# pnlybubbles/LumillyRender

Hardware: NVIDIA B200
Metric: Msamples/s (higher is better)
Workload: dtype f32

## Files before the change

lumillyrender_b200/csrc/api.cpp:

```cpp
#include <cuda_runtime.h>

#include <algorithm>
#include <chrono>
#include <cmath>
#include <cstdio>
#include <cstdlib>
#include <cstring>
#include <memory>
#include <mutex>
#include <string>
#include <system_error>
#include <thread>
#include <vector>

#include "common.h"
#include "kernels.h"

namespace lr {

thread_local std::string g_error;
void set_error(const std::string& s) { g_error = s; }
int fail(int code, const std::string& s) { g_error = s; return code; }

static int g_device = -1;
// ... 20 lines not shown
  return e;
}
static void dev_free(void* p) { if (p) cudaFreeAsync(p, 0); }

struct OnDevice {
  int prev = -1;
  explicit OnDevice(int device) {
    int cur = -1;
    if (cudaGetDevice(&cur) == cudaSuccess && cur != device && cudaSetDevice(device) == cudaSuccess) prev = cur;
  }
  ~OnDevice() { if (prev >= 0) cudaSetDevice(prev); }
  OnDevice(const OnDevice&) = delete;
  OnDevice& operator=(const OnDevice&) = delete;
};

static inline float4 mk4(float x, float y, float z, float w) { float4 r; r.x = x; r.y = y; r.z = z; r.w = w; return r; }
static inline float as_float(int32_t i) { float f; std::memcpy(&f, &i, 4); return f; }

}

using namespace lr;

struct LrScene {
  DevScene dev{};
  std::vector<void*> allocs;
  uint64_t h2d_bytes = 0;
  size_t block_bytes = 0;
  int width = 0, height = 0;
  unsigned long long* d_counters = nullptr;
  mutable float* d_film = nullptr; mutable size_t film_floats = 0;
  mutable float* d_film_sq = nullptr; mutable size_t film_sq_floats = 0;
  mutable float* d_partial = nullptr; mutable size_t partial_floats = 0;
  mutable float* d_partial_sq = nullptr; mutable size_t partial_sq_floats = 0;
  mutable uint64_t acc_samples = 0;
  mutable int acc_launches = 0;
  mutable int last_splits = 1;
  mutable float acc_kernel_ms = 0.0f;
  mutable cudaEvent_t ev0 = nullptr, ev1 = nullptr;
  mutable bool ev_pending = false;
  bool has_ggx = false;
  int device = 0, sm_count = 1;
};

extern "C" {

int lr_abi_version(void) { return LR_ABI_VERSION; }
const char* lr_last_error(void) { return g_error.c_str(); }

static int setup_device(int device, int* sm_count) {
  cudaDeviceProp prop;
  const cudaError_t e = cudaGetDeviceProperties(&prop, device);
  if (e != cudaSuccess) return fail(LR_ERR_NO_DEVICE, std::string("cudaGetDeviceProperties: ") + cudaGetErrorString(e));
  *sm_count = std::max(prop.multiProcessorCount, 1);
  cudaMemPool_t pool;
  if (cudaDeviceGetDefaultMemPool(&pool, device) == cudaSuccess) {
    unsigned long long keep = ~0ull;
    cudaMemPoolSetAttribute(pool, cudaMemPoolAttrReleaseThreshold, &keep);
  }
  return LR_OK;
}

int lr_init(int device) {
  int n = 0;
  cudaError_t e = cudaGetDeviceCount(&n);
  if (e != cudaSuccess || n <= 0)
    return fail(LR_ERR_NO_DEVICE, std::string("no CUDA device available (") + (e != cudaSuccess ? cudaGetErrorString(e) : "count = 0") +
// ... 175 lines not shown
    dv.bvh_hi[k] = d->n_nodes > 0 ? std::fmax(d->nodes[0].f[3 + k], d->nodes[0].f[9 + k]) : 0.0f;
  }
  dv.emission_area = area;
  dv.sky_type = d->sky.type;
  dv.sky_color[0] = d->sky.color[0]; dv.sky_color[1] = d->sky.color[1]; dv.sky_color[2] = d->sky.color[2];
  dv.sky_height = d->sky.height;
  dv.sky_longitude_offset = d->sky.longitude_offset;
  dv.cam = d->camera;
  s->width = d->camera.width; s->height = d->camera.height;
  for (int i = 0; i < d->n_materials; i++) s->has_ggx = s->has_ggx || d->materials[i].type == LR_MAT_GGX;
  guard.s = nullptr;
  *out = s;
  return LR_OK;
}

static int lr_scene_create_body(const LrSceneDesc* d, LrScene** out) {
  if (!d || !out) return fail(LR_ERR_INVALID, "null argument");
  *out = nullptr;
  if (int rc = validate_desc(*d)) return rc;
  if (int rc = ensure_device()) return rc;
  return scene_create(d, g_device, g_sm_count, out);
}
int lr_scene_create(const LrSceneDesc* d, LrScene** out) { LR_GUARDED(lr_scene_create_body(d, out)); }

void lr_scene_destroy(LrScene* s) {
  if (!s) return;
  if (s->ev_pending && s->ev1) cudaEventSynchronize(s->ev1);
  const OnDevice on(s->device);
  for (void* p : s->allocs) dev_free(p);
  dev_free(s->d_film);
  dev_free(s->d_film_sq);
  dev_free(s->d_partial);
  dev_free(s->d_partial_sq);
  if (s->ev0) cudaEventDestroy(s->ev0);
  if (s->ev1) cudaEventDestroy(s->ev1);
  delete s;
}

int lr_scene_bytes(const LrScene* s, uint64_t* h2d_bytes) {
  if (!s || !h2d_bytes) return fail(LR_ERR_INVALID, "null argument");
  *h2d_bytes = s->h2d_bytes;
  return LR_OK;
}

struct FilmShard { int index, count; };

static int resolve_params(const LrScene* s, const LrRenderParams* p, DevParams& dp, const FilmShard* shard = nullptr) {
  if (!s || !p) return fail(LR_ERR_INVALID, "null argument");
  if (p->integrator != LR_INTEGRATOR_PT && p->integrator != LR_INTEGRATOR_PT_DIRECT)
    return fail(LR_ERR_INVALID, "Unknown integrator type");
  if (p->spp_count <= 0 || p->spp_begin < 0) return fail(LR_ERR_INVALID, "spp range must be non-empty and non-negative");
  if (p->depth < 0 || p->depth_limit < 0) return fail(LR_ERR_INVALID, "depth and depth_limit must be >= 0");
  dp.integrator = p->integrator;
  dp.spp_begin = p->spp_begin; dp.spp_count = p->spp_count;
  dp.depth = p->depth; dp.depth_limit = p->depth_limit; dp.no_direct_emitter = p->no_direct_emitter ? 1 : 0;
  dp.seed = p->seed;
  if (p->crop_w > 0) {
    if (p->crop_h <= 0 || p->crop_x < 0 || p->crop_y < 0 || p->crop_x + p->crop_w > s->width || p->crop_y + p->crop_h > s->height)
      return fail(LR_ERR_INVALID, "crop window outside the film");
    dp.crop_x = p->crop_x; dp.crop_y = p->crop_y; dp.crop_w = p->crop_w; dp.crop_h = p->crop_h;
  } else {
    dp.crop_x = 0; dp.crop_y = 0; dp.crop_w = s->width; dp.crop_h = s->height;
  }
  dp.tiles_x = (dp.crop_w + 7) / 8; dp.tiles_y = (dp.crop_h + 3) / 4;
  int splits = shard ? 1 : p->splits;
  if (const char* e_splits = std::getenv("LR_SPLITS"); e_splits && !shard) splits = std::atoi(e_splits);
  if (splits <= 0) {
    const long long px_threads = (long long)dp.tiles_x * dp.tiles_y * 32;
    const long long target = 2LL * s->sm_count * 2048;
    splits = (int)std::min<long long>((target + px_threads - 1) / px_threads, std::max(1, p->spp_count / 4));
  }
  splits = std::max(1, std::min(splits, p->spp_count));
  const size_t px = (size_t)dp.crop_w * dp.crop_h;
  while (splits > 1 && px * 3 * sizeof(float) * splits > (1ull << 30)) splits--;
  dp.splits = splits;
  dp.shard = shard ? shard->index : 0;
  dp.n_shards = shard ? shard->count : 1;
  dp.unit_tiles = shard_tile_count(dp.tiles_x * dp.tiles_y, dp.shard, dp.n_shards);
  const char* e_di = std::getenv("LR_DEFER_ITERS");
  const char* e_dt = std::getenv("LR_DEFER_THRESH");
  dp.defer_iters = e_di ? std::max(1, std::atoi(e_di)) : 3;
  dp.defer_thresh = e_dt ? std::max(1, std::min(32, std::atoi(e_dt))) : 12;
  const char* e_org = std::getenv("LR_ORGANISATION");
  dp.organisation = !e_org ? 0 : (std::strcmp(e_org, "persistent") == 0 ? 1 : (std::strcmp(e_org, "pool") == 0 ? 2 : 0));

  return LR_OK;
}

static int ensure_scratch(float** buf, size_t* have, size_t need) {
  if (*have >= need) return LR_OK;
  dev_free(*buf);
  *buf = nullptr; *have = 0;
  LR_CUDA(dev_alloc((void**)buf, need * sizeof(float)));
  *have = need;
  return LR_OK;
}

static uint64_t shard_pixels(const DevParams& dp) {
  if (dp.n_shards == 1) return (uint64_t)dp.crop_w * dp.crop_h;
  uint64_t n = 0;
  for (int j = 0; j < dp.unit_tiles; j++) {
    const int t = shard_tile(j, dp.shard, dp.n_shards), tx = t % dp.tiles_x, ty = t / dp.tiles_x;
    n += (uint64_t)std::min(8, dp.crop_w - 8 * tx) * (uint64_t)std::min(4, dp.crop_h - 4 * ty);
  }
  return n;
}

static int accumulate(const LrScene* s, const LrRenderParams* p, float* d_sum, float* d_sumsq, void* cuda_stream, const FilmShard* shard) {
  if (!s) return fail(LR_ERR_INVALID, "null argument");
  const OnDevice on(s->device);
  DevParams dp;
  if (int rc = resolve_params(s, p, dp, shard)) return rc;
  if (!d_sum) return fail(LR_ERR_INVALID, "d_sum is null");
  cudaStream_t st = (cudaStream_t)cuda_stream;
  const size_t n = (size_t)dp.crop_w * dp.crop_h * 3;
  float* ksum = d_sum; float* ksq = d_sumsq;
  if (s->ev_pending) {
    float ms = 0.0f;
    if (cudaEventSynchronize(s->ev1) == cudaSuccess && cudaEventElapsedTime(&ms, s->ev0, s->ev1) == cudaSuccess) s->acc_kernel_ms += ms;
    s->ev_pending = false;
  }
  if (dp.unit_tiles == 0) return LR_OK;
  if (dp.splits > 1) {
    if (int rc = ensure_scratch(&s->d_partial, &s->partial_floats, n * dp.splits)) return rc;
    ksum = s->d_partial;
    if (d_sumsq) {
      if (int rc = ensure_scratch(&s->d_partial_sq, &s->partial_sq_floats, n * dp.splits)) return rc;
      ksq = s->d_partial_sq;
    }
  }
  LR_CUDA(cudaEventRecord(s->ev0, st));
  {
    unsigned int* next_unit = reinterpret_cast<unsigned int*>(s->d_counters + C_NEXT_UNIT);
    LR_CUDA(cudaMemsetAsync(next_unit, 0, sizeof(unsigned long long), st));
    LR_CUDA(launch_render_persistent(s->dev, dp, s->has_ggx, p->count_traversal != 0, ksum, d_sumsq ? ksq : nullptr, s->d_counters, next_unit,
                                     std::max(s->sm_count, 1), st));
    s->acc_launches++;
  }
  if (dp.splits > 1) {
    LR_CUDA(launch_reduce_splits(d_sum, s->d_partial, n, dp.splits, st));
    s->acc_launches++;
    if (d_sumsq) { LR_CUDA(launch_reduce_splits(d_sumsq, s->d_partial_sq, n, dp.splits, st)); s->acc_launches++; }
  }
  LR_CUDA(cudaEventRecord(s->ev1, st));
  s->ev_pending = true;
  s->acc_samples += shard_pixels(dp) * (uint64_t)dp.spp_count;
  s->last_splits = dp.splits;
  return LR_OK;
}

int lr_render_accumulate_device(const LrScene* s, const LrRenderParams* p, float* d_sum, float* d_sumsq, void* cuda_stream) {
  return accumulate(s, p, d_sum, d_sumsq, cuda_stream, nullptr);
}

int lr_stats_fetch(const LrScene* s, void* cuda_stream, LrStats* stats) {
  if (!s || !stats) return fail(LR_ERR_INVALID, "null argument");
  const OnDevice on(s->device);
  cudaStream_t st = (cudaStream_t)cuda_stream;
  LR_CUDA(cudaStreamSynchronize(st));
  if (s->ev_pending) {
    float ms = 0.0f;
    LR_CUDA(cudaEventSynchronize(s->ev1));
    LR_CUDA(cudaEventElapsedTime(&ms, s->ev0, s->ev1));
    s->acc_kernel_ms += ms;
    s->ev_pending = false;
  }
  unsigned long long c[C_COUNT];
  LR_CUDA(cudaMemcpy(c, s->d_counters, sizeof(c), cudaMemcpyDeviceToHost));
  LR_CUDA(cudaMemset(s->d_counters, 0, sizeof(c)));
  std::memset(stats, 0, sizeof(*stats));
  stats->rays = c[C_RAYS]; stats->nonfinite_samples = c[C_NONFINITE]; stats->gate_retraces = c[C_RETRACE];
  stats->nodes_visited = c[C_NODES]; stats->tris_tested = c[C_TRIS]; stats->spheres_tested = c[C_SPHERES];
  stats->flat_tris_tested = c[C_FLAT_TRIS]; stats->flat_boxes_tested = c[C_FLAT_BOXES];
  stats->samples = s->acc_samples; stats->kernel_ms = s->acc_kernel_ms; stats->launches = s->acc_launches; stats->splits = s->last_splits;
  s->acc_samples = 0; s->acc_kernel_ms = 0.0f; s->acc_launches = 0;
  return LR_OK;
}

int lr_render(const LrScene* s, const LrRenderParams* p, float* out_rgb, float* out_sumsq, LrStats* stats) {
  if (!s) return fail(LR_ERR_INVALID, "null argument");
  const OnDevice on(s->device);
  DevParams dp;
  if (int rc = resolve_params(s, p, dp)) return rc;
  if (!out_rgb) return fail(LR_ERR_INVALID, "out_rgb is null");
  const size_t n = (size_t)dp.crop_w * dp.crop_h * 3;
  if (int rc = ensure_scratch(&s->d_film, &s->film_floats, n)) return rc;
  if (out_sumsq) if (int rc = ensure_scratch(&s->d_film_sq, &s->film_sq_floats, n)) return rc;
  float *d_sum = s->d_film, *d_sq = out_sumsq ? s->d_film_sq : nullptr;
  int rc = LR_OK;
  do {
    if (cudaMemsetAsync(d_sum, 0, n * sizeof(float), 0) != cudaSuccess) { rc = fail(LR_ERR_CUDA, "cudaMemsetAsync failed"); break; }
    if (out_sumsq && cudaMemsetAsync(d_sq, 0, n * sizeof(float), 0) != cudaSuccess) { rc = fail(LR_ERR_CUDA, "cudaMemsetAsync failed"); break; }
    LrStats dummy;
    if (stats == nullptr) stats = &dummy;
    if ((rc = lr_stats_fetch(s, nullptr, stats)) != LR_OK) break;
    if ((rc = lr_render_accumulate_device(s, p, d_sum, d_sq, nullptr)) != LR_OK) break;
    cudaError_t e = launch_scale(d_sum, n, (float)dp.spp_count, 0);
    if (e != cudaSuccess) { rc = fail(LR_ERR_CUDA, std::string("scale: ") + cudaGetErrorString(e)); break; }
    if ((rc = lr_stats_fetch(s, nullptr, stats)) != LR_OK) break;
    stats->launches += 1;
    e = cudaMemcpy(out_rgb, d_sum, n * sizeof(float), cudaMemcpyDeviceToHost);
    if (e == cudaSuccess && out_sumsq) e = cudaMemcpy(out_sumsq, d_sq, n * sizeof(float), cudaMemcpyDeviceToHost);
// ... 646 lines not shown
```

lumillyrender_b200/csrc/device_scene.h:

```cpp
#pragma once
#include <cuda_runtime.h>
#include <stdint.h>
#include "../../include/lumilly.h"

namespace lr {

constexpr int kStackDepth = 64;
constexpr int kBlockThreads = 128;

struct DevScene {
  const float4* nodes;
  const float4* tris;
  const float4* tri_box;
  const float4* tri_n;
  const float4* spheres;
  const int2* sphere_meta;
  const float4* mats;
  const float* emitter_cdf;
  const float4* emitters;
  const float4* sky_pixels;
  int n_nodes, n_tris, n_spheres, n_emitters;
  int n_bvh_tris;
  float bvh_lo[3], bvh_hi[3];
  float emission_area;
  int sky_type;
  float sky_color[3];
  int sky_height;
  float sky_longitude_offset;
  LrCamera cam;
};

struct DevParams {
  int integrator;
  int spp_begin, spp_count;
  int depth, depth_limit, no_direct_emitter;
  unsigned long long seed;
  int crop_x, crop_y, crop_w, crop_h;
  int splits;
  int tiles_x, tiles_y;
  int shard, n_shards;
  int unit_tiles;
  int defer_iters, defer_thresh;
  int organisation;
};

__host__ __device__ inline int shard_of_tile(int tile, int n_shards) { return tile % n_shards; }
__host__ __device__ inline int shard_tile(int j, int shard, int n_shards) { return j * n_shards + shard; }
__host__ __device__ inline int shard_tile_count(int n_tiles, int shard, int n_shards) {
  return shard < n_tiles ? (n_tiles - shard + n_shards - 1) / n_shards : 0;
}
__host__ __device__ inline int shard_device(int shard, int n_devices) { return shard % n_devices; }
__host__ __device__ inline unsigned int render_units(const DevParams& p) { return (unsigned int)p.unit_tiles * 32u * (unsigned int)p.splits; }

enum CounterSlot { C_RAYS = 0, C_NONFINITE = 1, C_NODES = 2, C_TRIS = 3, C_SPHERES = 4, C_RETRACE = 5, C_FLAT_TRIS = 6, C_NEXT_UNIT = 7, C_FLAT_BOXES = 8, C_COUNT = 9 };

}
```

lumillyrender_b200/csrc/path_vertex.inc:

```
      bool need_new = false;
      bool fetch_unit = false;

      if (ready) {
        if (flags & F_HAS_RAY) {
          int depth = flags & F_DEPTH_MASK;
          bool allow_emission = (flags & F_ALLOW_EMISSION) != 0;
          bool has_shadow_next = false;
          const F3 d = d0;
          if (NR == 2 && (flags & F_HAS_SHADOW)) {
            PV_LOAD_SHADOW();
            if (id1 != -1 && fabsf(t1 - q_dist) <= kEPS) {
              const Surface lf = surface_at(sc, o, d1, t1, id1);
              const float light_cos = dot(-d1, lf.n);
              if (light_cos > 0.0f) {
                const Mat lm = load_mat(sc, lf.mat);
                const float g_term = q_point_cos * light_cos / q_sqr;
                const F3 l_i = lm.emissive ? lm.emission : f3(0.0f, 0.0f, 0.0f);
                const F3 direct = q_brdf * l_i * g_term / q_pdf;
                L = L + q_T * (q_prr != 1.0f ? direct / q_prr : direct);
              }
            }
          }
          bool finish = false;
          if (id0 == -1) {
// ... 55 lines not shown
              float pdf;
              mat_sample(m, wo, sf.n, rng, wi, pdf);
              F3 f_bsdf = f3(0, 0, 0);
#pragma unroll 1
              for (int k = (NR == 2 && has_shadow_next) ? 0 : 1; k < 2; k++) {
                const F3 f = mat_brdf(m, wo, k == 0 ? nee_dir : wi, k == 0 ? pn : sf.n, sf.pos);
                if (k == 0) { q_brdf = f; PV_STORE_QBRDF(); } else f_bsdf = f;
              }
              const F3 coef = mat_coef(m, wo, sf.n, t);
              const float c = dot(wi, sf.n);
              T = T * (f_bsdf * coef * c / pdf);
              if (prr != 1.0f) T = T / prr;
              o = sf.pos;
              d0 = wi;
              if (NR == 2 && has_shadow_next) d1 = nee_dir;
              depth++;
            }
          }
          if (finish) {
            PV_LOAD_FILM();
            const F3 e = (L * cam_g) * cam_w;
            if (!(isfinite(e.x) && isfinite(e.y) && isfinite(e.z))) n_nonfinite++;
            sum = sum + e;
            if (want_sumsq) sumsq = sumsq + e * e;
            un.y += 1;
            need_new = true;
          }
          flags = (flags & ~(F_DEPTH_MASK | F_ALLOW_EMISSION | F_HAS_SHADOW)) | (depth & F_DEPTH_MASK) |
                  (allow_emission ? F_ALLOW_EMISSION : 0) | (has_shadow_next ? F_HAS_SHADOW : 0);
        } else {
          need_new = true;
        }

        if (need_new && (!(flags & F_HAS_UNIT) || un.y >= un.z)) {
          if (flags & F_HAS_UNIT) {
            const size_t pi = (size_t)un.x, n_px = (size_t)p.crop_w * p.crop_h;
            if (p.splits == 1) {
              out_sum[3 * pi + 0] = sum.x; out_sum[3 * pi + 1] = sum.y; out_sum[3 * pi + 2] = sum.z;
              if (want_sumsq) { out_sumsq[3 * pi + 0] = sumsq.x; out_sumsq[3 * pi + 1] = sumsq.y; out_sumsq[3 * pi + 2] = sumsq.z; }
            } else {
              float* ps = out_sum + 3 * (n_px * un.w + pi);
              ps[0] = sum.x; ps[1] = sum.y; ps[2] = sum.z;
              if (want_sumsq) { float* pq = out_sumsq + 3 * (n_px * un.w + pi); pq[0] = sumsq.x; pq[1] = sumsq.y; pq[2] = sumsq.z; }
            }
          }
          fetch_unit = true;
        }
      }

      {
        bool need = fetch_unit;
        while (true) {
          const unsigned m = __ballot_sync(kFull, need);
          if (m == 0u) break;
          const int leader = __ffs(m) - 1;
          unsigned int base = 0;
          if (lane == leader) base = atomicAdd(next_unit, (unsigned int)__popc(m));
          base = __shfl_sync(kFull, base, leader);
          if (need) {
            const unsigned int u = base + (unsigned int)__popc(m & lanemask_lt());
            if (u >= n_units) {
              alive = false;
              need = false;
            } else {
              int lx, ly, split;
              if (decode_unit(p, u, lx, ly, split)) {
                const int per = p.spp_count / p.splits, rem = p.spp_count % p.splits;
                un.x = ly * p.crop_w + lx;
                un.y = p.spp_begin + split * per + min(split, rem);
                un.z = un.y + per + (split < rem ? 1 : 0);
                un.w = split;
                flags |= F_HAS_UNIT;
                sum = f3(0.0f, 0.0f, 0.0f);
                sumsq = f3(0.0f, 0.0f, 0.0f);
                if (p.splits == 1) {
                  const float* ps = out_sum + 3 * (size_t)un.x;
                  sum = f3(ps[0], ps[1], ps[2]);
                  if (want_sumsq) { const float* pq = out_sumsq + 3 * (size_t)un.x; sumsq = f3(pq[0], pq[1], pq[2]); }
                }
                need = false;
              }
            }
          }
        }
      }

      const bool go = ready && alive;
      if (go && need_new) {
        const int lx = un.x % p.crop_w, ly = un.x / p.crop_w;
        const int x = p.crop_x + lx, y = p.crop_y + ly;
        const unsigned int pixel = (unsigned int)(y * sc.cam.width + x);
        rng.seed(p.seed, pixel, (unsigned int)un.y);
        camera_sample_rng(sc.cam, x, y, rng, o, d0, cam_g, cam_w);
        T = f3(1.0f, 1.0f, 1.0f);
        L = f3(0.0f, 0.0f, 0.0f);
        flags = (flags & ~(F_DEPTH_MASK | F_HAS_SHADOW)) | F_ALLOW_EMISSION | F_HAS_RAY;
        PV_STORE_FILM();
      }
#pragma unroll 1
      for (int r = 0; r < NR; r++) {
        const bool on = go && (r == 0 || (flags & F_HAS_SHADOW));
        if (!__any_sync(kFull, on)) continue;
        if (on) {
          const F3 d = r == 0 ? d0 : d1;
          const F3 inv = f3(1.0f / d.x, 1.0f / d.y, 1.0f / d.z);
          float t = 3.0e38f;
          int id = -1;
          flat_hits<COUNT>(sc, flat, o, d, inv, t, id, tc);
          n_rays++;
          const bool pd = TREE && sc.n_nodes > 0 && bvh_bounds_hit(sc, o, inv, t < 3.0e38f ? t * 1.0001f + 1e-4f : 3.0e38f);
          if (r == 0) { t0 = t; id0 = id; pend0 = pd; } else { t1 = t; id1 = id; pend1 = pd; }
        }
      }
```

lumillyrender_b200/csrc/persistent.cuh:

```cuda
#pragma once
#include <algorithm>

#include "device_path.cuh"
#include "kernels.h"

namespace lr {

namespace pk {

constexpr unsigned kFull = 0xffffffffu;
enum { F_DEPTH_MASK = 0xffff, F_ALLOW_EMISSION = 1 << 16, F_HAS_RAY = 1 << 17, F_HAS_SHADOW = 1 << 18, F_HAS_UNIT = 1 << 20 };

LR_DEV unsigned lanemask_lt() { unsigned m; asm("mov.u32 %0, %%lanemask_lt;" : "=r"(m)); return m; }
LR_DEV unsigned int warp_sum_u(unsigned int v) { return __reduce_add_sync(kFull, v); }

LR_DEV bool decode_unit(const DevParams& p, unsigned int u, int& lx, int& ly, int& split) {
  const unsigned int per_split = (unsigned int)p.unit_tiles * 32u;
  split = (int)(u / per_split);
  const unsigned int r = u % per_split;
  const unsigned int tile = (unsigned int)shard_tile((int)(r >> 5), p.shard, p.n_shards), lane = r & 31u;
  lx = (int)(tile % p.tiles_x) * 8 + (int)(lane & 7u);
  ly = (int)(tile / p.tiles_x) * 4 + (int)(lane >> 3);
  return lx < p.crop_w && ly < p.crop_h;
}

template <bool COUNT>
__device__ __noinline__ void trace_strict(const DevScene& sc, F3 o, F3 d, float* t, int* id, TraceCounters* tc) {
  trace<COUNT>(sc, o, d, *t, *id, *tc);
}

}

#ifndef LR_MB_PT_TREE
#define LR_MB_PT_TREE 6
#endif
#ifndef LR_MB_PT_FLAT
#define LR_MB_PT_FLAT 8
#endif
#ifndef LR_MB_PTD_TREE
#define LR_MB_PTD_TREE 16
#endif
#ifndef LR_MB_PTD_FLAT
#define LR_MB_PTD_FLAT 4
#endif
template <int INTEGRATOR, bool TREE>
struct MinBlocks {
  static constexpr int value = INTEGRATOR == LR_INTEGRATOR_PT_DIRECT ? (TREE ? LR_MB_PTD_TREE : LR_MB_PTD_FLAT) : (TREE ? LR_MB_PT_TREE : LR_MB_PT_FLAT);
};

template <int INTEGRATOR, bool TREE, bool COUNT, int BUILD>
__global__ void __launch_bounds__(kBlockThreads, MinBlocks<INTEGRATOR, TREE>::value)
render_persistent_kernel(const __grid_constant__ DevScene sc, const __grid_constant__ DevParams p, float* __restrict__ out_sum,
                         float* __restrict__ out_sumsq, unsigned long long* __restrict__ counters, unsigned int* __restrict__ next_unit) {
  using namespace pk;
  constexpr int NR = INTEGRATOR == LR_INTEGRATOR_PT_DIRECT ? 2 : 1;
  const int lane = (int)(threadIdx.x & 31);
  const unsigned int n_units = render_units(p);
  const bool want_sumsq = out_sumsq != nullptr;
  __shared__ __align__(16) float4 flat_tab[kFlatListFloat4];
  __shared__ __align__(8) unsigned long long flat_bar;
  const FlatList flat = stage_flat_list(sc, flat_tab, &flat_bar);

  F3 o = f3(0, 0, 0), T = f3(1, 1, 1), L = f3(0, 0, 0), sum = f3(0, 0, 0), sumsq = f3(0, 0, 0);
  F3 d0 = f3(0, 0, 1), d1 = f3(0, 0, 1);
  float t0 = 3.0e38f, t1 = 3.0e38f;
  int id0 = -1, id1 = -1;
  bool pend0 = false, pend1 = false;
  float cam_g = 1.0f, cam_w = 1.0f;
  int4 un = make_int4(0, 0, 0, 0);
  Pcg rng;
  rng.state = 0;
  F3 q_T = f3(0, 0, 0), q_brdf = f3(0, 0, 0);
  float q_prr = 1.0f, q_point_cos = 0.0f, q_dist = 0.0f, q_sqr = 1.0f, q_pdf = 1.0f;
  int flags = 0;
  bool alive = true;
  unsigned int n_nonfinite = 0, n_retrace = 0, n_rays = 0;
  TraceCounters tc;
  tc.nodes = tc.tris = tc.spheres = tc.flat_tris = tc.flat_boxes = 0;

  while (true) {
    for (int it = 0; it < p.defer_iters; it++) {
      const bool ready = alive && !(pend0 || pend1);
      if (!__any_sync(kFull, ready)) break;
// ... 22 lines not shown
        int id = r == 0 ? id0 : id1;
        bvh_traverse_unified<COUNT>(sc, o, d, inv, t, id, tc);
        if (id >= 0 && id < sc.n_bvh_tris && !bvh_hit_is_gated(sc, o, inv, id)) {
          trace_strict<COUNT>(sc, o, d, &t, &id, &tc);
          n_retrace++;
        }
        if (r == 0) { t0 = t; id0 = id; pend0 = false; } else { t1 = t; id1 = id; pend1 = false; }
      }
    }
    if (!__any_sync(kFull, alive)) break;
  }

  n_rays = warp_sum_u(n_rays);
  n_nonfinite = warp_sum_u(n_nonfinite);
  n_retrace = warp_sum_u(n_retrace);
  if (COUNT) {
    tc.nodes = warp_sum_u(tc.nodes); tc.tris = warp_sum_u(tc.tris); tc.spheres = warp_sum_u(tc.spheres);
    tc.flat_tris = warp_sum_u(tc.flat_tris); tc.flat_boxes = warp_sum_u(tc.flat_boxes);
  }
  if (lane == 0) {
    if (n_rays) atomicAdd(counters + C_RAYS, (unsigned long long)n_rays);
    if (n_nonfinite) atomicAdd(counters + C_NONFINITE, (unsigned long long)n_nonfinite);
    if (n_retrace) atomicAdd(counters + C_RETRACE, (unsigned long long)n_retrace);
    if (COUNT) {
      atomicAdd(counters + C_NODES, (unsigned long long)tc.nodes);
      atomicAdd(counters + C_TRIS, (unsigned long long)tc.tris);
      atomicAdd(counters + C_SPHERES, (unsigned long long)tc.spheres);
      atomicAdd(counters + C_FLAT_TRIS, (unsigned long long)tc.flat_tris);
      atomicAdd(counters + C_FLAT_BOXES, (unsigned long long)tc.flat_boxes);
    }
  }
}

template <int INTEGRATOR, bool TREE, bool COUNT, int BUILD>
cudaError_t launch_persistent_one(const DevScene& sc, const DevParams& p, float* out_sum, float* out_sumsq,
                                  unsigned long long* counters, unsigned int* next_unit, int sm_count, cudaStream_t stream) {
  int nb = 0;
  if (cudaOccupancyMaxActiveBlocksPerMultiprocessor(&nb, render_persistent_kernel<INTEGRATOR, TREE, COUNT, BUILD>, kBlockThreads, 0) !=
          cudaSuccess || nb <= 0) nb = 4;
  const long long units = render_units(p);
  const long long want = (units + kBlockThreads - 1) / kBlockThreads;
  const unsigned int blocks = (unsigned int)std::max<long long>(1, std::min<long long>(want, (long long)nb * sm_count));
  render_persistent_kernel<INTEGRATOR, TREE, COUNT, BUILD><<<blocks, kBlockThreads, 0, stream>>>(sc, p, out_sum, out_sumsq, counters, next_unit);
  return cudaGetLastError();
}

}
```

lumillyrender_b200/csrc/pool.cuh:

```cuda
#pragma once
#include <algorithm>

#include "device_path.cuh"
#include "kernels.h"
#include "persistent.cuh"

namespace lr {

#ifndef LR_POOL_SLOTS
#define LR_POOL_SLOTS 64
#endif
#ifndef LR_POOL_SLOTS_PTD
#define LR_POOL_SLOTS_PTD 48
#endif
#ifndef LR_POOL_BSTART
#define LR_POOL_BSTART 32
#endif
#ifndef LR_PMB_PT_TREE
#define LR_PMB_PT_TREE 6
#endif
#ifndef LR_PMB_PTD_TREE
#define LR_PMB_PTD_TREE 6
#endif

// ... 21 lines not shown
__host__ __device__ constexpr int warp_words(bool want_sumsq) { return words_per_slot<INTEGRATOR>(want_sumsq) * slots<INTEGRATOR>() + 32; }

template <int N>
LR_DEV int select_take(int* list, int lane, unsigned (&words)[N], int quota, int rot) {
  const unsigned lt = pk::lanemask_lt();
  const unsigned bit = 1u << lane;
  int base = 0;
#pragma unroll
  for (int r = 0; r < N; r++) {
    if (r != rot) continue;
#pragma unroll
    for (int k = 0; k < N; k++) {
      const int i = (k + r) % N;
      const unsigned w = words[i];
      const int rank = base + __popc(w & lt);
      const bool mine = (w & bit) != 0u && rank < quota;
      if (mine) list[rank] = i * 32 + lane;
      words[i] = w & ~__ballot_sync(pk::kFull, mine);
      base += __popc(w);
    }
  }
  __syncwarp();
  return min(base, quota);
}

}

template <int INTEGRATOR, bool TREE>
struct PoolMinBlocks {
  static_assert(TREE, "the pool kernel is built for scenes with a BVH only (persistent_inst.cu)");
  static constexpr int value = INTEGRATOR == LR_INTEGRATOR_PT_DIRECT ? LR_PMB_PTD_TREE : LR_PMB_PT_TREE;
};

template <int INTEGRATOR, bool TREE, bool COUNT, int BUILD>
__global__ void __launch_bounds__(kBlockThreads, PoolMinBlocks<INTEGRATOR, TREE>::value)
render_pool_kernel(const __grid_constant__ DevScene sc, const __grid_constant__ DevParams p, float* __restrict__ out_sum,
                   float* __restrict__ out_sumsq, unsigned long long* __restrict__ counters, unsigned int* __restrict__ next_unit) {
  using namespace pk;
  using namespace pl;
  constexpr int NR = INTEGRATOR == LR_INTEGRATOR_PT_DIRECT ? 2 : 1;
  constexpr int NS = slots<INTEGRATOR>();
  constexpr int kWords = mask_words<INTEGRATOR>();
  __shared__ __align__(16) float4 flat_tab[kFlatListFloat4];
  __shared__ __align__(8) unsigned long long flat_bar;
  const FlatList flat = stage_flat_list(sc, flat_tab, &flat_bar);
  extern __shared__ float pool_smem[];
  const int lane = (int)(threadIdx.x & 31);
  const unsigned int n_units = render_units(p);
  const bool want_sumsq = out_sumsq != nullptr;
  float* const pool = pool_smem + (threadIdx.x >> 5) * warp_words<INTEGRATOR>(want_sumsq);
  int* const list = (int*)(pool + words_per_slot<INTEGRATOR>(want_sumsq) * NS);
  constexpr int W_SQ = NR == 2 ? (int)W_PTD_COUNT : (int)W_PT_COUNT;
#define SLF(w) pool[(w) * NS + s]
#define SLI(w) ((int*)pool)[(w) * NS + s]

  for (int s = lane; s < NS; s += 32) SLI(W_FLAGS) = 0;
  __syncwarp();

  unsigned pend[NR * kWords], dead[kWords];
#pragma unroll
  for (int i = 0; i < NR * kWords; i++) pend[i] = 0u;
#pragma unroll
  for (int i = 0; i < kWords; i++) dead[i] = (i + 1) * 32 <= NS ? 0u : ~0u << (NS - i * 32);
  unsigned int n_nonfinite = 0, n_retrace = 0, n_rays = 0;
  TraceCounters tc;
  tc.nodes = tc.tris = tc.spheres = tc.flat_tris = tc.flat_boxes = 0;
  int rot_a = 0, rot_b = 0;

  while (true) {
    unsigned rdy[kWords];
    int nA = 0, nB = 0;
#pragma unroll
    for (int i = 0; i < kWords; i++) {
      rdy[i] = ~(pend[i] | (NR == 2 ? pend[(NR - 1) * kWords + i] : 0u) | dead[i]);
      nA += __popc(rdy[i]);
    }
#pragma unroll
    for (int i = 0; i < NR * kWords; i++) nB += __popc(pend[i]);
    if (nA + nB == 0) break;

    if (!TREE || !(nB >= LR_POOL_BSTART || nB >= nA)) {
      const int n_sel = select_take<kWords>(list, lane, rdy, 32, rot_a);
      rot_a = rot_a + 1 == kWords ? 0 : rot_a + 1;
      const bool ready = lane < n_sel;
      const int s = ready ? list[lane] : 0;
      __syncwarp();
      bool alive = true;
      bool pend0 = false, pend1 = false;

      F3 o = f3(0, 0, 0), T = f3(1, 1, 1), L = f3(0, 0, 0), sum = f3(0, 0, 0), sumsq = f3(0, 0, 0);
      F3 d0 = f3(0, 0, 1), d1 = f3(0, 0, 1);
      float t0 = 3.0e38f, t1 = 3.0e38f;
      int id0 = -1, id1 = -1;
      float cam_g = 1.0f, cam_w = 1.0f;
      int4 un = make_int4(0, 0, 0, 0);
      Pcg rng;
      rng.state = 0;
      F3 q_T = f3(0, 0, 0), q_brdf = f3(0, 0, 0);
      float q_prr = 1.0f, q_point_cos = 0.0f, q_dist = 0.0f, q_sqr = 1.0f, q_pdf = 1.0f;
      int flags = 0;
      if (ready) {
        o = f3(SLF(W_OX), SLF(W_OY), SLF(W_OZ));
        d0 = f3(SLF(W_DX), SLF(W_DY), SLF(W_DZ));
        t0 = SLF(W_T0); id0 = SLI(W_ID0);
        T = f3(SLF(W_TX), SLF(W_TY), SLF(W_TZ));
        L = f3(SLF(W_LX), SLF(W_LY), SLF(W_LZ));
        rng.state = (unsigned long long)(unsigned int)SLI(W_RNGLO) | ((unsigned long long)(unsigned int)SLI(W_RNGHI) << 32);
        flags = SLI(W_FLAGS);
      }
#define PV_LOAD_SHADOW()                                                                                                  \
  do {                                                                                                                    \
    d1 = f3(SLF(W_D1X), SLF(W_D1Y), SLF(W_D1Z));                                                                          \
    t1 = SLF(W_T1); id1 = SLI(W_ID1);                                                                                     \
    q_T = f3(SLF(W_QTX), SLF(W_QTY), SLF(W_QTZ));                                                                         \
// ... 19 lines not shown
    SLF(W_CAMG) = cam_g; SLF(W_CAMW) = cam_w;                                                                             \
    SLI(W_UNX) = un.x; SLI(W_UNY) = un.y; SLI(W_UNZ) = un.z; SLI(W_UNW) = un.w;                                           \
    if (want_sumsq) { SLF(W_SQ) = sumsq.x; SLF(W_SQ + 1) = sumsq.y; SLF(W_SQ + 2) = sumsq.z; }                            \
  } while (0)

#include "path_vertex.inc"

#undef PV_LOAD_SHADOW
#undef PV_STORE_SHADOW
#undef PV_STORE_QBRDF
#undef PV_LOAD_FILM
#undef PV_STORE_FILM
      if (go) {
        SLF(W_OX) = o.x; SLF(W_OY) = o.y; SLF(W_OZ) = o.z;
        SLF(W_DX) = d0.x; SLF(W_DY) = d0.y; SLF(W_DZ) = d0.z;
        SLF(W_T0) = t0; SLI(W_ID0) = id0;
        SLF(W_TX) = T.x; SLF(W_TY) = T.y; SLF(W_TZ) = T.z;
        SLF(W_LX) = L.x; SLF(W_LY) = L.y; SLF(W_LZ) = L.z;
        SLI(W_RNGLO) = (int)(unsigned int)rng.state; SLI(W_RNGHI) = (int)(unsigned int)(rng.state >> 32);
        SLI(W_FLAGS) = flags;
        if (NR == 2 && (flags & F_HAS_SHADOW)) {
          SLF(W_D1X) = d1.x; SLF(W_D1Y) = d1.y; SLF(W_D1Z) = d1.z;
          SLF(W_T1) = t1; SLI(W_ID1) = id1;
        }
      }
      const unsigned bit = 1u << (s & 31);
      const int w = s >> 5;
#pragma unroll
      for (int i = 0; i < kWords; i++) {
        pend[i] |= __reduce_or_sync(kFull, (go && pend0 && w == i) ? bit : 0u);
        if (NR == 2) pend[(NR - 1) * kWords + i] |= __reduce_or_sync(kFull, (go && pend1 && w == i) ? bit : 0u);
        dead[i] |= __reduce_or_sync(kFull, (ready && !alive && w == i) ? bit : 0u);
      }
    } else {
      const int n_sel = select_take<NR * kWords>(list, lane, pend, 32, rot_b);
      rot_b = rot_b + 1 == NR * kWords ? 0 : rot_b + 1;
      if (lane < n_sel) {
        const int item = list[lane];
        const int s = item % (32 * kWords);
        const bool shadow = NR == 2 && item >= 32 * kWords;
        const F3 o = f3(SLF(W_OX), SLF(W_OY), SLF(W_OZ));
        const F3 d = shadow ? f3(SLF(W_D1X), SLF(W_D1Y), SLF(W_D1Z)) : f3(SLF(W_DX), SLF(W_DY), SLF(W_DZ));
        const F3 inv = f3(1.0f / d.x, 1.0f / d.y, 1.0f / d.z);
        float t = shadow ? SLF(W_T1) : SLF(W_T0);
        int id = shadow ? SLI(W_ID1) : SLI(W_ID0);
        bvh_traverse_unified<COUNT>(sc, o, d, inv, t, id, tc);
        if (id >= 0 && id < sc.n_bvh_tris && !bvh_hit_is_gated(sc, o, inv, id)) {
          trace_strict<COUNT>(sc, o, d, &t, &id, &tc);
          n_retrace++;
        }
        if (shadow) { SLF(W_T1) = t; SLI(W_ID1) = id; } else { SLF(W_T0) = t; SLI(W_ID0) = id; }
      }
    }
    __syncwarp();
  }
#undef SLF
#undef SLI

  n_rays = warp_sum_u(n_rays);
  n_nonfinite = warp_sum_u(n_nonfinite);
  n_retrace = warp_sum_u(n_retrace);
  if (COUNT) {
    tc.nodes = warp_sum_u(tc.nodes); tc.tris = warp_sum_u(tc.tris); tc.spheres = warp_sum_u(tc.spheres);
    tc.flat_tris = warp_sum_u(tc.flat_tris); tc.flat_boxes = warp_sum_u(tc.flat_boxes);
  }
  if (lane == 0) {
    if (n_rays) atomicAdd(counters + C_RAYS, (unsigned long long)n_rays);
    if (n_nonfinite) atomicAdd(counters + C_NONFINITE, (unsigned long long)n_nonfinite);
    if (n_retrace) atomicAdd(counters + C_RETRACE, (unsigned long long)n_retrace);
    if (COUNT) {
      atomicAdd(counters + C_NODES, (unsigned long long)tc.nodes);
      atomicAdd(counters + C_TRIS, (unsigned long long)tc.tris);
      atomicAdd(counters + C_SPHERES, (unsigned long long)tc.spheres);
      atomicAdd(counters + C_FLAT_TRIS, (unsigned long long)tc.flat_tris);
      atomicAdd(counters + C_FLAT_BOXES, (unsigned long long)tc.flat_boxes);
    }
  }
}

template <int INTEGRATOR, bool TREE, bool COUNT, int BUILD>
cudaError_t launch_pool_one(const DevScene& sc, const DevParams& p, float* out_sum, float* out_sumsq, unsigned long long* counters,
                            unsigned int* next_unit, int sm_count, cudaStream_t stream) {
  auto kernel = render_pool_kernel<INTEGRATOR, TREE, COUNT, BUILD>;
  const size_t smem = (size_t)(kBlockThreads / 32) * pl::warp_words<INTEGRATOR>(out_sumsq != nullptr) * sizeof(float);
  cudaError_t e = cudaFuncSetAttribute(kernel, cudaFuncAttributeMaxDynamicSharedMemorySize, (int)smem);
  if (e != cudaSuccess) return e;
  int nb = 0;
  if (cudaOccupancyMaxActiveBlocksPerMultiprocessor(&nb, kernel, kBlockThreads, smem) != cudaSuccess || nb <= 0) nb = 2;
  const long long units = render_units(p);
  const long long per_block = (long long)(kBlockThreads / 32) * pl::slots<INTEGRATOR>();
  const long long want = (units + per_block - 1) / per_block;
  const unsigned int blocks = (unsigned int)std::max<long long>(1, std::min<long long>(want, (long long)nb * sm_count));
  kernel<<<blocks, kBlockThreads, smem, stream>>>(sc, p, out_sum, out_sumsq, counters, next_unit);
  return cudaGetLastError();
}

}
```

Baseline: 1362.

## Chain per-pixel sample chunks with device-side release/acquire instead of split reductions

When only one split is chosen, each pixel's samples are divided into chunks that run as separate work units. Each unit waits on a per-pixel done counter, using acquire and release atomics, before it accumulates into the film. The aim is to expose more parallel units for small images without the partial-buffer reduction pass. The cost is a per-pixel counter memset, spin-waiting lanes, and a timeout path that abandons stalled units.

After: 1428 (median of 6 runs). 4.9% higher.

```diff
diff --git a/lumillyrender_b200/csrc/api.cpp b/lumillyrender_b200/csrc/api.cpp
--- a/lumillyrender_b200/csrc/api.cpp
+++ b/lumillyrender_b200/csrc/api.cpp
@@ -76,6 +76,7 @@
   mutable float* d_film_sq = nullptr; mutable size_t film_sq_floats = 0;
   mutable float* d_partial = nullptr; mutable size_t partial_floats = 0;
   mutable float* d_partial_sq = nullptr; mutable size_t partial_sq_floats = 0;
+  mutable unsigned int* d_done = nullptr; mutable size_t done_words = 0;
   mutable uint64_t acc_samples = 0;
   mutable int acc_launches = 0;
   mutable int last_splits = 1;
@@ -317,6 +318,7 @@
   dev_free(s->d_film_sq);
   dev_free(s->d_partial);
   dev_free(s->d_partial_sq);
+  dev_free(s->d_done);
   if (s->ev0) cudaEventDestroy(s->ev0);
   if (s->ev1) cudaEventDestroy(s->ev1);
   delete s;
@@ -359,6 +361,9 @@
   const size_t px = (size_t)dp.crop_w * dp.crop_h;
   while (splits > 1 && px * 3 * sizeof(float) * splits > (1ull << 30)) splits--;
   dp.splits = splits;
+  const char* e_chunk = std::getenv("LR_CHUNK_SPP");
+  dp.chunk_spp = !e_chunk ? 0 : (std::atoi(e_chunk) > 0 ? std::atoi(e_chunk) : -1);
+  dp.done = nullptr;
   dp.shard = shard ? shard->index : 0;
   dp.n_shards = shard ? shard->count : 1;
   dp.unit_tiles = shard_tile_count(dp.tiles_x * dp.tiles_y, dp.shard, dp.n_shards);
@@ -415,6 +420,13 @@
     }
   }
   LR_CUDA(cudaEventRecord(s->ev0, st));
+  if (dp.splits == 1 && dp.chunk_spp >= 0) {
+    const size_t n_px = (size_t)dp.crop_w * dp.crop_h;
+    static_assert(sizeof(unsigned int) == sizeof(float), "the done counters share the float scratch allocator");
+    if (int rc = ensure_scratch((float**)&s->d_done, &s->done_words, n_px)) return rc;
+    LR_CUDA(cudaMemsetAsync(s->d_done, 0, n_px * sizeof(unsigned int), st));
+    dp.done = s->d_done;
+  }
   {
     unsigned int* next_unit = reinterpret_cast<unsigned int*>(s->d_counters + C_NEXT_UNIT);
     LR_CUDA(cudaMemsetAsync(next_unit, 0, sizeof(unsigned long long), st));
@@ -453,6 +465,9 @@
   unsigned long long c[C_COUNT];
   LR_CUDA(cudaMemcpy(c, s->d_counters, sizeof(c), cudaMemcpyDeviceToHost));
   LR_CUDA(cudaMemset(s->d_counters, 0, sizeof(c)));
+  if (c[C_WAIT_ABANDONED])
+    return fail(LR_ERR_CUDA, std::to_string(c[C_WAIT_ABANDONED]) + " chained render unit(s) waited more than " + std::to_string(kChainWaitMs / 1000) +
+                                 " s for the previous chunk of their pixel and were abandoned: the image is incomplete");
   std::memset(stats, 0, sizeof(*stats));
   stats->rays = c[C_RAYS]; stats->nonfinite_samples = c[C_NONFINITE]; stats->gate_retraces = c[C_RETRACE];
   stats->nodes_visited = c[C_NODES]; stats->tris_tested = c[C_TRIS]; stats->spheres_tested = c[C_SPHERES];
diff --git a/lumillyrender_b200/csrc/device_scene.h b/lumillyrender_b200/csrc/device_scene.h
--- a/lumillyrender_b200/csrc/device_scene.h
+++ b/lumillyrender_b200/csrc/device_scene.h
@@ -42,6 +42,8 @@
   int unit_tiles;
   int defer_iters, defer_thresh;
   int organisation;
+  unsigned int* done;
+  int chunk_spp;
 };
 
 __host__ __device__ inline int shard_of_tile(int tile, int n_shards) { return tile % n_shards; }
@@ -51,7 +53,31 @@
 }
 __host__ __device__ inline int shard_device(int shard, int n_devices) { return shard % n_devices; }
 __host__ __device__ inline unsigned int render_units(const DevParams& p) { return (unsigned int)p.unit_tiles * 32u * (unsigned int)p.splits; }
+__host__ __device__ inline bool decode_unit(const DevParams& p, unsigned int u, int& lx, int& ly, int& split) {
+  const unsigned int per_split = (unsigned int)p.unit_tiles * 32u;
+  split = (int)(u / per_split);
+  const unsigned int r = u % per_split;
+  const unsigned int tile = (unsigned int)shard_tile((int)(r >> 5), p.shard, p.n_shards), lane = r & 31u;
+  lx = (int)(tile % p.tiles_x) * 8 + (int)(lane & 7u);
+  ly = (int)(tile / p.tiles_x) * 4 + (int)(lane >> 3);
+  return lx < p.crop_w && ly < p.crop_h;
+}
+__host__ __device__ inline void split_samples(const DevParams& p, int split, int& begin, int& end) {
+  const int per = p.spp_count / p.splits, rem = p.spp_count % p.splits;
+  begin = p.spp_begin + split * per + (split < rem ? split : rem);
+  end = begin + per + (split < rem ? 1 : 0);
+}
 
-enum CounterSlot { C_RAYS = 0, C_NONFINITE = 1, C_NODES = 2, C_TRIS = 3, C_SPHERES = 4, C_RETRACE = 5, C_FLAT_TRIS = 6, C_NEXT_UNIT = 7, C_FLAT_BOXES = 8, C_COUNT = 9 };
+__host__ __device__ inline int chain_chunks(const DevParams& p, long long slots) {
+  if (p.chunk_spp > 0) return (p.spp_count + p.chunk_spp - 1) / p.chunk_spp;
+  const long long px = (long long)p.unit_tiles * 32;
+  if (px < slots) return 1;
+  const long long want = (64 * slots + px - 1) / px, most = p.spp_count / 64;
+  return (int)(want < most ? want : most > 1 ? most : 1);
+}
+
+enum CounterSlot { C_RAYS = 0, C_NONFINITE = 1, C_NODES = 2, C_TRIS = 3, C_SPHERES = 4, C_RETRACE = 5, C_FLAT_TRIS = 6, C_NEXT_UNIT = 7, C_FLAT_BOXES = 8,
+                   C_WAIT_ABANDONED = 9, C_COUNT = 10 };
+constexpr unsigned int kChainWaitMs = 20000;
 
 }
diff --git a/lumillyrender_b200/csrc/path_vertex.inc b/lumillyrender_b200/csrc/path_vertex.inc
--- a/lumillyrender_b200/csrc/path_vertex.inc
+++ b/lumillyrender_b200/csrc/path_vertex.inc
@@ -111,12 +111,13 @@
           need_new = true;
         }
 
-        if (need_new && (!(flags & F_HAS_UNIT) || un.y >= un.z)) {
+        if (need_new && !(CHAIN && (flags & F_WAIT)) && (!(flags & F_HAS_UNIT) || un.y >= un.z)) {
           if (flags & F_HAS_UNIT) {
             const size_t pi = (size_t)un.x, n_px = (size_t)p.crop_w * p.crop_h;
-            if (p.splits == 1) {
+            if (p.splits == 1 || CHAIN) {
               out_sum[3 * pi + 0] = sum.x; out_sum[3 * pi + 1] = sum.y; out_sum[3 * pi + 2] = sum.z;
               if (want_sumsq) { out_sumsq[3 * pi + 0] = sumsq.x; out_sumsq[3 * pi + 1] = sumsq.y; out_sumsq[3 * pi + 2] = sumsq.z; }
+              if (CHAIN) st_release(p.done + pi, (unsigned int)un.w + 1u);
             } else {
               float* ps = out_sum + 3 * (n_px * un.w + pi);
               ps[0] = sum.x; ps[1] = sum.y; ps[2] = sum.z;
@@ -144,15 +145,16 @@
             } else {
               int lx, ly, split;
               if (decode_unit(p, u, lx, ly, split)) {
-                const int per = p.spp_count / p.splits, rem = p.spp_count % p.splits;
                 un.x = ly * p.crop_w + lx;
-                un.y = p.spp_begin + split * per + min(split, rem);
-                un.z = un.y + per + (split < rem ? 1 : 0);
+                split_samples(p, split, un.y, un.z);
                 un.w = split;
                 flags |= F_HAS_UNIT;
                 sum = f3(0.0f, 0.0f, 0.0f);
                 sumsq = f3(0.0f, 0.0f, 0.0f);
-                if (p.splits == 1) {
+                if (CHAIN) {
+                  flags = (flags & ~(F_HAS_RAY | F_HAS_SHADOW)) | F_WAIT;
+                  sum.x = __uint_as_float(timer_ms());
+                } else if (p.splits == 1) {
                   const float* ps = out_sum + 3 * (size_t)un.x;
                   sum = f3(ps[0], ps[1], ps[2]);
                   if (want_sumsq) { const float* pq = out_sumsq + 3 * (size_t)un.x; sumsq = f3(pq[0], pq[1], pq[2]); }
@@ -164,21 +166,40 @@
         }
       }
 
+      bool waiting = false;
+      if (CHAIN && ready && alive && (flags & F_WAIT)) {
+        if (!fetch_unit) PV_LOAD_FILM();
+        const size_t pi = (size_t)un.x;
+        if (ld_acquire(p.done + pi) == (unsigned int)un.w) {
+          const float* ps = out_sum + 3 * pi;
+          sum = f3(ps[0], ps[1], ps[2]);
+          if (want_sumsq) { const float* pq = out_sumsq + 3 * pi; sumsq = f3(pq[0], pq[1], pq[2]); }
+          flags &= ~F_WAIT;
+        } else if (timer_ms() - __float_as_uint(sum.x) > kChainWaitMs) {
+          atomicAdd(counters + C_WAIT_ABANDONED, 1ull);
+          alive = false;
+        } else {
+          waiting = true;
+        }
+      }
+
       const bool go = ready && alive;
       if (go && need_new) {
-        const int lx = un.x % p.crop_w, ly = un.x / p.crop_w;
-        const int x = p.crop_x + lx, y = p.crop_y + ly;
-        const unsigned int pixel = (unsigned int)(y * sc.cam.width + x);
-        rng.seed(p.seed, pixel, (unsigned int)un.y);
-        camera_sample_rng(sc.cam, x, y, rng, o, d0, cam_g, cam_w);
-        T = f3(1.0f, 1.0f, 1.0f);
-        L = f3(0.0f, 0.0f, 0.0f);
-        flags = (flags & ~(F_DEPTH_MASK | F_HAS_SHADOW)) | F_ALLOW_EMISSION | F_HAS_RAY;
+        if (!waiting) {
+          const int lx = un.x % p.crop_w, ly = un.x / p.crop_w;
+          const int x = p.crop_x + lx, y = p.crop_y + ly;
+          const unsigned int pixel = (unsigned int)(y * sc.cam.width + x);
+          rng.seed(p.seed, pixel, (unsigned int)un.y);
+          camera_sample_rng(sc.cam, x, y, rng, o, d0, cam_g, cam_w);
+          T = f3(1.0f, 1.0f, 1.0f);
+          L = f3(0.0f, 0.0f, 0.0f);
+          flags = (flags & ~(F_DEPTH_MASK | F_HAS_SHADOW)) | F_ALLOW_EMISSION | F_HAS_RAY;
+        }
         PV_STORE_FILM();
       }
 #pragma unroll 1
       for (int r = 0; r < NR; r++) {
-        const bool on = go && (r == 0 || (flags & F_HAS_SHADOW));
+        const bool on = go && !waiting && (r == 0 || (flags & F_HAS_SHADOW));
         if (!__any_sync(kFull, on)) continue;
         if (on) {
           const F3 d = r == 0 ? d0 : d1;
diff --git a/lumillyrender_b200/csrc/persistent.cuh b/lumillyrender_b200/csrc/persistent.cuh
--- a/lumillyrender_b200/csrc/persistent.cuh
+++ b/lumillyrender_b200/csrc/persistent.cuh
@@ -1,5 +1,6 @@
 #pragma once
 #include <algorithm>
+#include <cuda/atomic>
 
 #include "device_path.cuh"
 #include "kernels.h"
@@ -9,19 +10,17 @@
 namespace pk {
 
 constexpr unsigned kFull = 0xffffffffu;
-enum { F_DEPTH_MASK = 0xffff, F_ALLOW_EMISSION = 1 << 16, F_HAS_RAY = 1 << 17, F_HAS_SHADOW = 1 << 18, F_HAS_UNIT = 1 << 20 };
+enum { F_DEPTH_MASK = 0xffff, F_ALLOW_EMISSION = 1 << 16, F_HAS_RAY = 1 << 17, F_HAS_SHADOW = 1 << 18, F_HAS_UNIT = 1 << 20, F_WAIT = 1 << 21 };
 
 LR_DEV unsigned lanemask_lt() { unsigned m; asm("mov.u32 %0, %%lanemask_lt;" : "=r"(m)); return m; }
 LR_DEV unsigned int warp_sum_u(unsigned int v) { return __reduce_add_sync(kFull, v); }
 
-LR_DEV bool decode_unit(const DevParams& p, unsigned int u, int& lx, int& ly, int& split) {
-  const unsigned int per_split = (unsigned int)p.unit_tiles * 32u;
-  split = (int)(u / per_split);
-  const unsigned int r = u % per_split;
-  const unsigned int tile = (unsigned int)shard_tile((int)(r >> 5), p.shard, p.n_shards), lane = r & 31u;
-  lx = (int)(tile % p.tiles_x) * 8 + (int)(lane & 7u);
-  ly = (int)(tile / p.tiles_x) * 4 + (int)(lane >> 3);
-  return lx < p.crop_w && ly < p.crop_h;
+LR_DEV unsigned int ld_acquire(unsigned int* a) { return cuda::atomic_ref<unsigned int, cuda::thread_scope_device>(*a).load(cuda::memory_order_acquire); }
+LR_DEV void st_release(unsigned int* a, unsigned int v) { cuda::atomic_ref<unsigned int, cuda::thread_scope_device>(*a).store(v, cuda::memory_order_release); }
+LR_DEV unsigned int timer_ms() {
+  unsigned long long t;
+  asm volatile("mov.u64 %0, %%globaltimer;" : "=l"(t));
+  return (unsigned int)(t >> 20);
 }
 
 template <bool COUNT>
@@ -48,7 +47,7 @@
   static constexpr int value = INTEGRATOR == LR_INTEGRATOR_PT_DIRECT ? (TREE ? LR_MB_PTD_TREE : LR_MB_PTD_FLAT) : (TREE ? LR_MB_PT_TREE : LR_MB_PT_FLAT);
 };
 
-template <int INTEGRATOR, bool TREE, bool COUNT, int BUILD>
+template <int INTEGRATOR, bool TREE, bool COUNT, int BUILD, bool CHAIN>
 __global__ void __launch_bounds__(kBlockThreads, MinBlocks<INTEGRATOR, TREE>::value)
 render_persistent_kernel(const __grid_constant__ DevScene sc, const __grid_constant__ DevParams p, float* __restrict__ out_sum,
                          float* __restrict__ out_sumsq, unsigned long long* __restrict__ counters, unsigned int* __restrict__ next_unit) {
@@ -137,16 +136,29 @@
   }
 }
 
+inline DevParams chained(const DevParams& p, long long slots) {
+  DevParams q = p;
+  if (q.done) {
+    q.splits = chain_chunks(p, slots);
+    if (q.splits <= 1) { q.splits = 1; q.done = nullptr; }
+  }
+  return q;
+}
+
 template <int INTEGRATOR, bool TREE, bool COUNT, int BUILD>
 cudaError_t launch_persistent_one(const DevScene& sc, const DevParams& p, float* out_sum, float* out_sumsq,
                                   unsigned long long* counters, unsigned int* next_unit, int sm_count, cudaStream_t stream) {
   int nb = 0;
-  if (cudaOccupancyMaxActiveBlocksPerMultiprocessor(&nb, render_persistent_kernel<INTEGRATOR, TREE, COUNT, BUILD>, kBlockThreads, 0) !=
+  if (cudaOccupancyMaxActiveBlocksPerMultiprocessor(&nb, render_persistent_kernel<INTEGRATOR, TREE, COUNT, BUILD, false>, kBlockThreads, 0) !=
           cudaSuccess || nb <= 0) nb = 4;
-  const long long units = render_units(p);
+  const DevParams q = chained(p, (long long)nb * sm_count * kBlockThreads);
+  const long long units = render_units(q);
   const long long want = (units + kBlockThreads - 1) / kBlockThreads;
   const unsigned int blocks = (unsigned int)std::max<long long>(1, std::min<long long>(want, (long long)nb * sm_count));
-  render_persistent_kernel<INTEGRATOR, TREE, COUNT, BUILD><<<blocks, kBlockThreads, 0, stream>>>(sc, p, out_sum, out_sumsq, counters, next_unit);
+  if (q.done)
+    render_persistent_kernel<INTEGRATOR, TREE, COUNT, BUILD, true><<<blocks, kBlockThreads, 0, stream>>>(sc, q, out_sum, out_sumsq, counters, next_unit);
+  else
+    render_persistent_kernel<INTEGRATOR, TREE, COUNT, BUILD, false><<<blocks, kBlockThreads, 0, stream>>>(sc, q, out_sum, out_sumsq, counters, next_unit);
   return cudaGetLastError();
 }
 
diff --git a/lumillyrender_b200/csrc/pool.cuh b/lumillyrender_b200/csrc/pool.cuh
--- a/lumillyrender_b200/csrc/pool.cuh
+++ b/lumillyrender_b200/csrc/pool.cuh
@@ -77,7 +77,7 @@
   static constexpr int value = INTEGRATOR == LR_INTEGRATOR_PT_DIRECT ? LR_PMB_PTD_TREE : LR_PMB_PT_TREE;
 };
 
-template <int INTEGRATOR, bool TREE, bool COUNT, int BUILD>
+template <int INTEGRATOR, bool TREE, bool COUNT, int BUILD, bool CHAIN>
 __global__ void __launch_bounds__(kBlockThreads, PoolMinBlocks<INTEGRATOR, TREE>::value)
 render_pool_kernel(const __grid_constant__ DevScene sc, const __grid_constant__ DevParams p, float* __restrict__ out_sum,
                    float* __restrict__ out_sumsq, unsigned long long* __restrict__ counters, unsigned int* __restrict__ next_unit) {
@@ -103,6 +103,7 @@
   __syncwarp();
 
   unsigned pend[NR * kWords], dead[kWords];
+  bool stalled = false;
 #pragma unroll
   for (int i = 0; i < NR * kWords; i++) pend[i] = 0u;
 #pragma unroll
@@ -124,7 +125,7 @@
     for (int i = 0; i < NR * kWords; i++) nB += __popc(pend[i]);
     if (nA + nB == 0) break;
 
-    if (!TREE || !(nB >= LR_POOL_BSTART || nB >= nA)) {
+    if (!TREE || !(nB >= LR_POOL_BSTART || nB >= nA || (CHAIN && stalled && nB > 0))) {
       const int n_sel = select_take<kWords>(list, lane, rdy, 32, rot_a);
       rot_a = rot_a + 1 == kWords ? 0 : rot_a + 1;
       const bool ready = lane < n_sel;
@@ -210,7 +211,9 @@
         if (NR == 2) pend[(NR - 1) * kWords + i] |= __reduce_or_sync(kFull, (go && pend1 && w == i) ? bit : 0u);
         dead[i] |= __reduce_or_sync(kFull, (ready && !alive && w == i) ? bit : 0u);
       }
+      if (CHAIN) stalled = __all_sync(kFull, !ready || waiting);
     } else {
+      if (CHAIN) stalled = false;
       const int n_sel = select_take<NR * kWords>(list, lane, pend, 32, rot_b);
       rot_b = rot_b + 1 == NR * kWords ? 0 : rot_b + 1;
       if (lane < n_sel) {
@@ -259,17 +262,20 @@
 template <int INTEGRATOR, bool TREE, bool COUNT, int BUILD>
 cudaError_t launch_pool_one(const DevScene& sc, const DevParams& p, float* out_sum, float* out_sumsq, unsigned long long* counters,
                             unsigned int* next_unit, int sm_count, cudaStream_t stream) {
-  auto kernel = render_pool_kernel<INTEGRATOR, TREE, COUNT, BUILD>;
+  auto kernel = render_pool_kernel<INTEGRATOR, TREE, COUNT, BUILD, false>;
+  auto kernel_chained = render_pool_kernel<INTEGRATOR, TREE, COUNT, BUILD, true>;
   const size_t smem = (size_t)(kBlockThreads / 32) * pl::warp_words<INTEGRATOR>(out_sumsq != nullptr) * sizeof(float);
   cudaError_t e = cudaFuncSetAttribute(kernel, cudaFuncAttributeMaxDynamicSharedMemorySize, (int)smem);
+  if (e == cudaSuccess) e = cudaFuncSetAttribute(kernel_chained, cudaFuncAttributeMaxDynamicSharedMemorySize, (int)smem);
   if (e != cudaSuccess) return e;
   int nb = 0;
   if (cudaOccupancyMaxActiveBlocksPerMultiprocessor(&nb, kernel, kBlockThreads, smem) != cudaSuccess || nb <= 0) nb = 2;
-  const long long units = render_units(p);
   const long long per_block = (long long)(kBlockThreads / 32) * pl::slots<INTEGRATOR>();
+  const DevParams q = chained(p, (long long)nb * sm_count * per_block);
+  const long long units = render_units(q);
   const long long want = (units + per_block - 1) / per_block;
   const unsigned int blocks = (unsigned int)std::max<long long>(1, std::min<long long>(want, (long long)nb * sm_count));
-  kernel<<<blocks, kBlockThreads, smem, stream>>>(sc, p, out_sum, out_sumsq, counters, next_unit);
+  (q.done ? kernel_chained : kernel)<<<blocks, kBlockThreads, smem, stream>>>(sc, q, out_sum, out_sumsq, counters, next_unit);
   return cudaGetLastError();
 }
 
```
